# xiuqhou/Salience-DETR

Hardware: AMD Instinct MI355X
Metric: images/s (whole node) + ms/encoder-layer, ResNet50 800x1333 (higher is better)
Workload: dtype bf16; 1 GPU; salience_detr_resnet50_800_1333 bf16 inference, batch=2 per MI355X: pyramid flatten + hierarchical salience filtering + 6-layer salience encoder (MSDA); batch_per_gpu=2, global_batch=2, parallelism=replicas, images sharded across GPUs, no data-path collective, hipgraph=True, hipgraph_nodes=44, hipgraph_memset_nodes=0, world_size=1, backend=none (single process)

## Files before the change

salience_detr_amd/csrc/salience_head.hip:

```cpp
#include <cstdlib>

#include "common.h"

#include "salience_head_core.h"

namespace sdetr {

__global__ void __launch_bounds__(512, 2) salience_head_stage1_x3_kernel(Stage1Args p)
{
    stage1_x3_body(p, (int)blockIdx.x, (int)blockIdx.y);
}

__global__ void __launch_bounds__(512, 2) salience_head_hoist_pyramid_kernel(Stage1Args p, PyramidSrc src, int s1_blocks)
{
    const int blk = (int)blockIdx.x;
    stage1_x3_body<true>(p, blk % s1_blocks, blk / s1_blocks, &src);
}

template <int RT, int WAVES = 4>
__global__ void __launch_bounds__(64 * WAVES, WAVES == 8 ? 2 : (RT == 2 ? 2 : 4)) salience_head_stage1_kernel(Stage1Args p)
{
    constexpr int TM = 32 * RT, THREADS = 64 * WAVES, CT = 8 / WAVES;
    static_assert(TM * 64 % THREADS == 0 && THREADS % TM == 0, "tile / block shape");
    extern __shared__ __attribute__((aligned(16))) float smem[];
    float *tile = smem;
    float *par = smem + TM * kXS;
    float *srow = par + kParRows * kC;
    const int tid = threadIdx.x, lane = tid & 63, wave = tid >> 6;
    const int b = blockIdx.y, blk = blockIdx.x;
    const int t0 = blk * TM;
    const int nvalid = min(TM, p.n - t0);
    const int n0 = wave * (32 * CT);
    const bool with_enc = p.w_enc != nullptr;

    WeightStream<CT, 4> ws;
    ws.start(with_enc ? p.w_enc : p.w1, kC, kC / 8, n0, lane);

    {
        const float *xb = p.x + (int64_t)b * p.x_batch_stride + (int64_t)t0 * p.x_row_stride;
        constexpr int NL = TM * 64 / THREADS;
        float4 v[NL];
#pragma unroll
        for (int i = 0; i < NL; ++i) {
            const int idx = tid + i * THREADS;
            const int r = idx >> 6, c4 = idx & 63;
            v[i] = *reinterpret_cast<const float4 *>(xb + (int64_t)min(r, nvalid - 1) * p.x_row_stride + c4 * 4);
        }
        if (tid < 256) {
            const int row = tid >> 6, c4 = tid & 63;
            const float *src0 = row == 0 ? p.b_enc : row == 1 ? p.g_enc : row == 2 ? p.beta_enc : p.g1;
            const float *src1 = row == 0 ? p.beta1 : p.b1;
            if (with_enc || row == 3) *reinterpret_cast<float4 *>(par + row * kC + c4 * 4) =
                                          *reinterpret_cast<const float4 *>(src0 + c4 * 4);
            if (row < 2) *reinterpret_cast<float4 *>(par + (4 + row) * kC + c4 * 4) =
                             *reinterpret_cast<const float4 *>(src1 + c4 * 4);
        }
        if (tid < TM) {
            float s = 0.f;
            const int t = min(t0 + tid, p.n - 1);
            if (p.row_scale) {
                s = p.row_scale[(int64_t)b * p.n + t];
            } else if (p.coarse) {
                const int y = t / p.w, x = t - y * p.w;
                const float sh = p.h > 1 ? (float)(p.ch - 1) / (float)(p.h - 1) : 0.f;
                const float sw = p.w > 1 ? (float)(p.cw - 1) / (float)(p.w - 1) : 0.f;
                const float fy = sh * (float)y, fx = sw * (float)x;
                const int y1 = (int)fy, x1 = (int)fx;
                const int yp = y1 < p.ch - 1 ? 1 : 0, xp = x1 < p.cw - 1 ? 1 : 0;
                const float ly = fy - (float)y1, lx = fx - (float)x1;
                const float hy = 1.f - ly, hx = 1.f - lx;
                const float *cm = p.coarse + (int64_t)b * p.ch * p.cw;
                s = hy * (hx * cm[y1 * p.cw + x1] + lx * cm[y1 * p.cw + x1 + xp]) +
                    ly * (hx * cm[(y1 + yp) * p.cw + x1] + lx * cm[(y1 + yp) * p.cw + x1 + xp]);
            }
            srow[tid] = s;
            if (tid == 0) srow[TM] = (p.row_scale || p.coarse) ? (p.alpha ? *p.alpha : 1.f) : 0.f;
        }
#pragma unroll
        for (int i = 0; i < NL; ++i) {
            const int idx = tid + i * THREADS;
            const int r = idx >> 6, c4 = idx & 63;
            *reinterpret_cast<float4 *>(tile + r * kXS + c4 * 4) = r < nvalid ? v[i] : make_float4(0.f, 0.f, 0.f, 0.f);
        }
    }
    __syncthreads();

    f32x16 acc[RT][CT];
    if (with_enc) {
        zero_acc(acc);
        block_gemm<kC, kXS, RT, CT, 4>(tile, ws, lane, acc);
        ws.start(p.w1, kC, kC / 8, n0, lane);
        __syncthreads();
#pragma unroll
        for (int ct = 0; ct < CT; ++ct) {
            const int c = n0 + 32 * ct + (lane & 31);
            const float bias = par[kParBEnc * kC + c];
#pragma unroll
            for (int rt = 0; rt < RT; ++rt)
#pragma unroll
                for (int i = 0; i < 16; ++i) tile[(32 * rt + acc_row(i, lane)) * kXS + c] = acc[rt][ct][i] + bias;
        }
        __syncthreads();
    }

    {
        constexpr int TPR = THREADS / TM, NV = kC / 4 / TPR, CS = 4 * TPR;
        const int r = tid / TPR, q = tid % TPR;
        float *row = tile + r * kXS + 4 * q;
        float4 v[NV];
#pragma unroll
        for (int i = 0; i < NV; ++i) v[i] = *reinterpret_cast<const float4 *>(row + CS * i);
        float mean, rstd;
        if (with_enc) {
            row_stats<NV, TPR>(v, p.eps_enc, mean, rstd);
#pragma unroll
            for (int i = 0; i < NV; ++i)
                v[i] = ln_apply(v[i], mean, rstd, *reinterpret_cast<const float4 *>(par + kParGEnc * kC + CS * i + 4 * q),
                                *reinterpret_cast<const float4 *>(par + kParBetaEnc * kC + CS * i + 4 * q));
            if (p.memory_out && r < nvalid) {
                float *mo = p.memory_out + (int64_t)b * p.mem_batch_stride + (int64_t)(t0 + r) * kC + 4 * q;
#pragma unroll
                for (int i = 0; i < NV; ++i) *reinterpret_cast<float4 *>(mo + CS * i) = v[i];
            }
        }
        const float s = srow[r], a = srow[TM];
        if (a != 0.f) {
#pragma unroll
            for (int i = 0; i < NV; ++i)
                v[i] = make_float4(v[i].x + v[i].x * s * a, v[i].y + v[i].y * s * a, v[i].z + v[i].z * s * a,
                                   v[i].w + v[i].w * s * a);
        }
        row_stats<NV, TPR>(v, p.eps1, mean, rstd);
#pragma unroll
        for (int i = 0; i < NV; ++i)
            *reinterpret_cast<float4 *>(row + CS * i) =
                ln_apply(v[i], mean, rstd, *reinterpret_cast<const float4 *>(par + kParG1 * kC + CS * i + 4 * q),
                         *reinterpret_cast<const float4 *>(par + kParBeta1 * kC + CS * i + 4 * q));
    }
    __syncthreads();

    zero_acc(acc);
    block_gemm<kC, kXS, RT, CT, 4>(tile, ws, lane, acc);
    if (n0 < kHalf) {
        float *zl = p.z_local + ((int64_t)b * p.n + t0) * kHalf;
#pragma unroll
        for (int ct = 0; ct < CT; ++ct) {
            const int c = n0 + 32 * ct + (lane & 31);
            const float bias = par[kParB1 * kC + c];
#pragma unroll
            for (int rt = 0; rt < RT; ++rt)
#pragma unroll
                for (int i = 0; i < 16; ++i) {
                    const int r = 32 * rt + acc_row(i, lane);
                    if (r < nvalid) zl[(int64_t)r * kHalf + c] = gelu_erf(acc[rt][ct][i] + bias);
                }
        }
    } else {
#pragma unroll
        for (int ct = 0; ct < CT; ++ct) {
            const int c = n0 + 32 * ct + (lane & 31);
            const float bias = par[kParB1 * kC + c];
            float s = 0.f;
#pragma unroll
            for (int rt = 0; rt < RT; ++rt)
#pragma unroll
                for (int i = 0; i < 16; ++i) {
                    const int r = 32 * rt + acc_row(i, lane);
                    s += r < nvalid ? gelu_erf(acc[rt][ct][i] + bias) : 0.f;
// ... 88 lines not shown
    const int64_t i = (int64_t)blockIdx.x * blockDim.x + threadIdx.x;
    if (i >= (int64_t)N * K) return;
    const int j = (int)(i & 3), h = (int)((i >> 2) & 1);
    const int64_t rest = i >> 3;
    const int n = (int)(rest % N), S = (int)(rest / N);
    out[i] = w[(int64_t)n * row_stride + 8 * S + 4 * h + j];
}

}

using namespace sdetr;

extern "C" int sdetr_pack_linear_f32(sdetr_stream_t stream, const float *weight, int64_t row_stride, int out_features,
                                     int in_features, float *packed)
{
    if (!weight || !packed) return fail("pack_linear: NULL pointer");
    if (out_features <= 0 || in_features <= 0 || in_features % 8 != 0)
        return fail("pack_linear: in_features must be a positive multiple of 8 (got %d x %d)", out_features, in_features);
    const int64_t total = (int64_t)out_features * in_features;
    hipLaunchKernelGGL(pack_linear_kernel, dim3((unsigned)((total + 255) / 256)), dim3(256), 0,
                       static_cast<hipStream_t>(stream), weight, row_stride, out_features, in_features, packed);
    return check_launch("pack_linear");
}

static int stage1_lds_bytes(int tm) { return (tm * kXS + kParRows * kC + tm + 4) * (int)sizeof(float); }

static int stage1_block_tokens(int batch_size, int tokens)
{
    static const int forced = [] { const char *e = ab_env("SDETR_HEAD_ROWTILES"); return e ? atoi(e) : 0; }();
    (void)batch_size; (void)tokens;
    return forced == 2 ? 64 : 32;
}

extern "C" int sdetr_salience_head_blocks(int batch_size, int tokens)
{
    if (tokens <= 0 || batch_size <= 0) return 0;
    const int tm = stage1_block_tokens(batch_size, tokens);
    return (tokens + tm - 1) / tm;
}

extern "C" int sdetr_salience_head_stage1(sdetr_stream_t stream, const float *x, int64_t x_batch_stride,
                                          int64_t x_row_stride, int batch_size, int tokens, int channels,
                                          const float *enc_weight_packed, const float *enc_bias,
                                          const float *enc_norm_weight, const float *enc_norm_bias, float enc_norm_eps,
                                          const float *row_scale, const float *coarse_score, int coarse_h, int coarse_w,
                                          int level_h, int level_w, const float *alpha, const float *norm_weight,
                                          const float *norm_bias, float norm_eps, const float *weight_packed,
                                          const float *bias, float *memory_out, int64_t memory_batch_stride,
                                          float *z_local, float *partial_sums)
{
    if (channels != kC) return fail("salience_head_stage1: built for embed_dim = hidden_dim = %d (got %d)", kC, channels);
    if (batch_size < 0 || tokens < 0) return fail("salience_head_stage1: negative size");
    if (batch_size == 0 || tokens == 0) return 0;
    if (!x || !norm_weight || !norm_bias || !weight_packed || !bias || !z_local || !partial_sums)
        return fail("salience_head_stage1: NULL pointer");
    if (enc_weight_packed && (!enc_bias || !enc_norm_weight || !enc_norm_bias))
        return fail("salience_head_stage1: enc_output parameters incomplete");
    if (row_scale && coarse_score) return fail("salience_head_stage1: give row_scale OR coarse_score");
    if (coarse_score && ((int64_t)level_h * level_w != tokens || coarse_h <= 0 || coarse_w <= 0))
        return fail("salience_head_stage1: level %dx%d does not cover %d tokens", level_h, level_w, tokens);
    if ((x_row_stride % 4) || (x_batch_stride % 4)) return fail("salience_head_stage1: rows must be 16-byte aligned");
    Stage1Args a;
    a.x = x; a.x_batch_stride = x_batch_stride; a.x_row_stride = x_row_stride;
    a.w_enc = reinterpret_cast<const float4 *>(enc_weight_packed);
    a.b_enc = enc_bias; a.g_enc = enc_norm_weight; a.beta_enc = enc_norm_bias; a.eps_enc = enc_norm_eps;
    a.row_scale = row_scale; a.coarse = coarse_score; a.ch = coarse_h; a.cw = coarse_w; a.h = level_h; a.w = level_w;
    a.alpha = alpha; a.g1 = norm_weight; a.beta1 = norm_bias; a.eps1 = norm_eps;
    a.w1 = reinterpret_cast<const float4 *>(weight_packed); a.b1 = bias;
    a.memory_out = enc_weight_packed ? memory_out : nullptr; a.mem_batch_stride = memory_batch_stride;
    a.z_local = z_local; a.partial = partial_sums; a.n = tokens; a.nblk = 0;

    hipStream_t s = static_cast<hipStream_t>(stream);
    if (stage1_block_tokens(batch_size, tokens) == 64) {
        static DeviceOnce lds_once;
        allow_dynamic_lds(salience_head_stage1_kernel<2, 4>, lds_once, (int)stage1_lds_bytes(64));
        a.nblk = (tokens + 63) / 64;
        hipLaunchKernelGGL((salience_head_stage1_kernel<2, 4>), dim3((unsigned)a.nblk, (unsigned)batch_size), dim3(kBlock),
                           (size_t)stage1_lds_bytes(64), s, a);
    } else {
        a.nblk = (tokens + 31) / 32;
        hipLaunchKernelGGL((salience_head_stage1_kernel<1, 8>), dim3((unsigned)a.nblk, (unsigned)batch_size), dim3(512),
                           (size_t)stage1_lds_bytes(32), s, a);
    }
    return check_launch("salience_head_stage1");
}

extern "C" int sdetr_pack_linear_bf16x3(sdetr_stream_t stream, const float *weight, int64_t row_stride, int out_features,
                                        int in_features, void *packed)
{
    if (!weight || !packed) return fail("pack_linear_bf16x3: NULL pointer");
    if (out_features <= 0 || in_features <= 0 || in_features % 16 != 0 || out_features % 32 != 0)
        return fail("pack_linear_bf16x3: [out,in] must be multiples of (32,16) (got %d x %d)", out_features, in_features);
    const int64_t total = (int64_t)out_features * in_features;
    hipLaunchKernelGGL(pack_linear_bf16x3_kernel, dim3((unsigned)((total + 255) / 256)), dim3(256), 0,
                       static_cast<hipStream_t>(stream), weight, row_stride, out_features, in_features,
                       static_cast<uint16_t *>(packed));
    return check_launch("pack_linear_bf16x3");
}

static int stage1_x3_lds_bytes() { return kX3Region + (kParRows * kC + 32 + 4) * (int)sizeof(float); }

extern "C" int sdetr_salience_head_stage1_x3(sdetr_stream_t stream, const float *x, int64_t x_batch_stride,
                                             int64_t x_row_stride, int batch_size, int tokens, int channels,
                                             const void *enc_weight_x3, const float *enc_bias,
                                             const float *enc_norm_weight, const float *enc_norm_bias, float enc_norm_eps,
                                             const float *row_scale, const float *coarse_score, int coarse_h, int coarse_w,
                                             int level_h, int level_w, const float *alpha, const float *norm_weight,
                                             const float *norm_bias, float norm_eps, const void *weight_x3,
                                             const float *bias, float *memory_out, int64_t memory_batch_stride,
                                             float *z_local, float *partial_sums)
{
    if (channels != kC) return fail("salience_head_stage1_x3: built for embed_dim = hidden_dim = %d (got %d)", kC, channels);
    if (batch_size < 0 || tokens < 0) return fail("salience_head_stage1_x3: negative size");
    if (batch_size == 0 || tokens == 0) return 0;
    if (!x || !norm_weight || !norm_bias || !weight_x3 || !bias || !z_local || !partial_sums)
        return fail("salience_head_stage1_x3: NULL pointer");
    if (enc_weight_x3 && (!enc_bias || !enc_norm_weight || !enc_norm_bias))
        return fail("salience_head_stage1_x3: enc_output parameters incomplete");
    if (row_scale && coarse_score) return fail("salience_head_stage1_x3: give row_scale OR coarse_score");
    if (coarse_score && ((int64_t)level_h * level_w != tokens || coarse_h <= 0 || coarse_w <= 0))
        return fail("salience_head_stage1_x3: level %dx%d does not cover %d tokens", level_h, level_w, tokens);
    if ((x_row_stride % 4) || (x_batch_stride % 4)) return fail("salience_head_stage1_x3: rows must be 16-byte aligned");
    if (stage1_block_tokens(batch_size, tokens) != 32)
        return fail("salience_head_stage1_x3: 32-token blocks only (unset SDETR_HEAD_ROWTILES)");
    Stage1Args a;
    a.x = x; a.x_batch_stride = x_batch_stride; a.x_row_stride = x_row_stride;
    a.w_enc = reinterpret_cast<const float4 *>(enc_weight_x3);
    a.b_enc = enc_bias; a.g_enc = enc_norm_weight; a.beta_enc = enc_norm_bias; a.eps_enc = enc_norm_eps;
    a.row_scale = row_scale; a.coarse = coarse_score; a.ch = coarse_h; a.cw = coarse_w; a.h = level_h; a.w = level_w;
    a.alpha = alpha; a.g1 = norm_weight; a.beta1 = norm_bias; a.eps1 = norm_eps;
    a.w1 = reinterpret_cast<const float4 *>(weight_x3); a.b1 = bias;
    a.memory_out = enc_weight_x3 ? memory_out : nullptr; a.mem_batch_stride = memory_batch_stride;
    a.z_local = z_local; a.partial = partial_sums; a.n = tokens; a.nblk = (tokens + 31) / 32;
    hipLaunchKernelGGL(salience_head_stage1_x3_kernel, dim3((unsigned)a.nblk, (unsigned)batch_size), dim3(512),
                       (size_t)stage1_x3_lds_bytes(), static_cast<hipStream_t>(stream), a);
    return check_launch("salience_head_stage1_x3");
}

extern "C" int sdetr_salience_head_hoist_pyramid_x3(
    sdetr_stream_t stream, int num_levels, const float *const *feats, const float *const *pos, const uint8_t *const *masks,
    const int *heights, const int *widths, const float *level_embeds, int batch_size, int channels, int spatial_size,
    uint8_t *mask_out, void *feat_act, void *pos_act, float *valid_ratios, const void *enc_weight_x3, const float *enc_bias,
    const float *enc_norm_weight, const float *enc_norm_bias, float enc_norm_eps, const float *norm_weight,
    const void *weight_x3, float *memory_out, int64_t memory_batch_stride, float *g_out, int64_t g_batch_stride,
    float *sigma_out, int64_t sigma_batch_stride)
{
    if (num_levels <= 0 || num_levels > kPyrMaxLevels) return fail("salience_head_hoist_pyramid_x3: 1..%d levels", kPyrMaxLevels);
    if (channels != kC) return fail("salience_head_hoist_pyramid_x3: built for embed_dim = hidden_dim = %d (got %d)", kC, channels);
    if (batch_size < 0 || spatial_size <= 0) return fail("salience_head_hoist_pyramid_x3: bad dims");
    if (!feats || !pos || !masks || !heights || !widths || !level_embeds || !mask_out || !feat_act || !pos_act)
        return fail("salience_head_hoist_pyramid_x3: null pointer");
    if (!enc_weight_x3 || !enc_bias || !enc_norm_weight || !enc_norm_bias || !norm_weight || !weight_x3 || !g_out || !sigma_out)
        return fail("salience_head_hoist_pyramid_x3: null pointer (head)");
    if ((g_batch_stride % 4) || g_batch_stride < (int64_t)spatial_size * kC || sigma_batch_stride < spatial_size ||
        (memory_out && ((memory_batch_stride % 4) || memory_batch_stride < (int64_t)spatial_size * kC)))
        return fail("salience_head_hoist_pyramid_x3: bad output batch strides");
    if (stage1_block_tokens(batch_size, spatial_size) != 32)
        return fail("salience_head_hoist_pyramid_x3: 32-token blocks only (unset SDETR_HEAD_ROWTILES)");
    PyramidSrc src{};
    src.levels = num_levels;
    int64_t start = 0;
    for (int l = 0; l < num_levels; ++l) {
        const int H = heights[l], W = widths[l];
        if (H <= 0 || W <= 0 || !feats[l] || !pos[l] || !masks[l]) return fail("salience_head_hoist_pyramid_x3: bad level %d", l);
        src.feat[l] = feats[l]; src.pos[l] = pos[l]; src.mask[l] = masks[l];
        src.H[l] = H; src.W[l] = W; src.start[l] = (int)start;
        src.box_wh[l] = 0.05f * (float)(1u << l);
        start += (int64_t)H * W;
        if (start > spatial_size || (int64_t)batch_size * kC * H * W > 0x7fffffffffffLL)
            return fail("salience_head_hoist_pyramid_x3: sizes out of range");
    }
    if (start != spatial_size)
        return fail("salience_head_hoist_pyramid_x3: spatial_size %d is not the pixel count %lld", spatial_size, (long long)start);
    for (int l = num_levels; l <= kPyrMaxLevels; ++l) src.start[l] = spatial_size;
    for (int l = 0; l + kPyrTileLevels < num_levels; ++l)
        if (src.start[l + kPyrTileLevels] / 32 == (src.start[l + 1] - 1) / 32)
            return fail("salience_head_hoist_pyramid_x3: more than %d levels inside one 32-token tile", kPyrTileLevels);
    if (batch_size == 0) return 0;
    src.level_embed = level_embeds;
    src.feat_act = reinterpret_cast<bf16_t *>(feat_act); src.pos_act = reinterpret_cast<bf16_t *>(pos_act);
    src.mask_out = mask_out; src.valid_ratios = valid_ratios;
    Stage1Args a;
    a.x = nullptr; a.x_batch_stride = 0; a.x_row_stride = 0;
    a.w_enc = reinterpret_cast<const float4 *>(enc_weight_x3);
    a.b_enc = enc_bias; a.g_enc = enc_norm_weight; a.beta_enc = enc_norm_bias; a.eps_enc = enc_norm_eps;
    a.row_scale = nullptr; a.coarse = nullptr; a.ch = a.cw = a.h = a.w = 0;
    a.alpha = nullptr; a.g1 = norm_weight; a.beta1 = norm_weight; a.eps1 = 0.f;
    a.w1 = reinterpret_cast<const float4 *>(weight_x3); a.b1 = norm_weight;
    a.memory_out = memory_out; a.mem_batch_stride = memory_batch_stride;
    a.z_local = nullptr; a.partial = nullptr; a.n = spatial_size; a.nblk = (spatial_size + 31) / 32;
    a.g_out = g_out; a.g_batch_stride = g_batch_stride; a.sigma_out = sigma_out; a.sigma_batch_stride = sigma_batch_stride;
    if ((int64_t)a.nblk * batch_size > 0x7fffffff) return fail("salience_head_hoist_pyramid_x3: too many tiles");
    static DeviceOnce lds_once;
    const int lds = kPyrLdsFloats * (int)sizeof(float);
    allow_dynamic_lds(salience_head_hoist_pyramid_kernel, lds_once, lds);
    hipLaunchKernelGGL(salience_head_hoist_pyramid_kernel, dim3((unsigned)(a.nblk * batch_size)), dim3(512), (size_t)lds,
                       static_cast<hipStream_t>(stream), a, src, a.nblk);
    return check_launch("salience_head_hoist_pyramid_x3");
}

extern "C" int sdetr_salience_head_const(sdetr_stream_t stream, const float *partial_sums, int batch_size, int tokens,
                                         const float *weight2, const float *bias2, float *const_workspace,
                                         float *score_min)
{
    if (batch_size < 0 || tokens < 0) return fail("salience_head_const: negative size");
    if (batch_size == 0 || tokens == 0) return 0;
    if (!partial_sums || !weight2 || !bias2 || !const_workspace) return fail("salience_head_const: NULL pointer");
    hipLaunchKernelGGL(salience_head_const_kernel, dim3((unsigned)batch_size), dim3(kHalf * kConstGroups), 0,
                       static_cast<hipStream_t>(stream), partial_sums, sdetr_salience_head_blocks(batch_size, tokens),
                       tokens, weight2, bias2, const_workspace, score_min);
    return check_launch("salience_head_const");
}

extern "C" int sdetr_salience_head_stage2(sdetr_stream_t stream, const float *z_local, const float *partial_sums,
                                          int batch_size, int tokens, const float *weight2, const float *bias2,
                                          const float *weight2_local_packed, const float *weight3_packed,
                                          const float *bias3, const float *weight4, const float *bias4,
                                          float *const_workspace, float *score, float *score_flat,
                                          int64_t score_flat_stride, float *score_min, const void *weight2_local_x3,
                                          int const_in_block)
{
    if (batch_size < 0 || tokens < 0) return fail("salience_head_stage2: negative size");
    if (batch_size == 0 || tokens == 0) return 0;
    if (!z_local || !partial_sums || !weight2 || !bias2 || (!weight2_local_packed && !weight2_local_x3) || !weight3_packed ||
        !bias3 || !weight4 || !bias4 || (!const_workspace && !const_in_block) || !score)
        return fail("salience_head_stage2: NULL pointer");
    const int nblk = (tokens + kTM - 1) / kTM;
    const int prow = sdetr_salience_head_blocks(batch_size, tokens);
    if (const_in_block && prow > kConstInBlockRows)
        return fail("salience_head_stage2: the constant in the block takes up to %d rows of partial sums (got %d)", kConstInBlockRows, prow);
    hipStream_t s = static_cast<hipStream_t>(stream);
    Stage2Args a;
    if (const_in_block) {
        a.partial = partial_sums; a.partial_rows = prow; a.w2 = weight2; a.b2 = bias2;
    } else {
        hipLaunchKernelGGL(salience_head_const_kernel, dim3((unsigned)batch_size), dim3(kHalf * kConstGroups), 0, s,
                           partial_sums, prow, tokens, weight2, bias2, const_workspace, score_min);
        int rc = check_launch("salience_head_const");
        if (rc) return rc;
    }
    a.z_local = z_local; a.cst = const_workspace;
    a.w2a = reinterpret_cast<const float4 *>(weight2_local_packed);
    a.w2a_x3 = weight2_local_x3;
    a.w3 = reinterpret_cast<const float4 *>(weight3_packed);
    a.b3 = bias3; a.w4 = weight4; a.b4 = bias4; a.score = score; a.score2 = score_flat;
    a.score2_stride = score_flat_stride; a.n = tokens; a.score_min = score_min;
    hipLaunchKernelGGL(salience_head_stage2_kernel, dim3((unsigned)nblk, (unsigned)batch_size), dim3(kBlock), 0, s, a);
    return check_launch("salience_head_stage2");
}
```

salience_detr_amd/csrc/salience_head_core.h:

```cpp
#pragma once
#include "common.h"

#pragma clang fp contract(off)

namespace sdetr {

constexpr int kC = 256;
constexpr int kHalf = 128;
constexpr int kTM = 64;
constexpr int kXS = kC + 4;
constexpr int kZS = kHalf + 4;

using f32x16 = __attribute__((ext_vector_type(16))) float;

__device__ __forceinline__ float erf_pos(float t)
{
    float p = 4.535823973128572e-05f;
    p = fmaf(p, t, -0.00044550452730618417f);
    p = fmaf(p, t, 0.0014894308988004923f);
    p = fmaf(p, t, 0.0007746480405330658f);
    p = fmaf(p, t, -0.028253698721528053f);
    p = fmaf(p, t, 0.14848162233829498f);
    p = fmaf(p, t, 0.9184163808822632f);
    p = fmaf(p, t, 1.6279085874557495f);
// ... 60 lines not shown
            if (S + PD < NS) {
#pragma unroll
                for (int ct = 0; ct < CT; ++ct)
                    ws.bq[u][ct] = __builtin_amdgcn_raw_buffer_load_b128(ws.rs, (int)(ws.lane_off + ct * 1024),
                                                                         (int)((S + PD) * ws.step), 0);
            }
#pragma unroll
            for (int rt = 0; rt < RT; ++rt) a[rt] = *reinterpret_cast<const float4 *>(ap + rt * 32 * XS + 8 * S);
            __builtin_amdgcn_sched_barrier(0);
#pragma unroll
            for (int rt = 0; rt < RT; ++rt)
#pragma unroll
                for (int ct = 0; ct < CT; ++ct) {
                    const float4 bf = make_float4(__uint_as_float(b[ct].x), __uint_as_float(b[ct].y),
                                                  __uint_as_float(b[ct].z), __uint_as_float(b[ct].w));
                    acc[rt][ct] = mfma4(a[rt], bf, acc[rt][ct]);
                }
        }
    }
}

template <int RT, int CT>
__device__ __forceinline__ void zero_acc(f32x16 (&acc)[RT][CT])
{
#pragma unroll
    for (int rt = 0; rt < RT; ++rt)
#pragma unroll
        for (int ct = 0; ct < CT; ++ct)
#pragma unroll
            for (int i = 0; i < 16; ++i) acc[rt][ct][i] = 0.f;
}

__device__ __forceinline__ int acc_row(int reg, int lane) { return (reg & 3) + 8 * (reg >> 2) + 4 * (lane >> 5); }

struct Stage1Args {
    const float *x;
    int64_t x_batch_stride, x_row_stride;
    const float4 *w_enc;
    const float *b_enc, *g_enc, *beta_enc;
    float eps_enc;
    const float *row_scale;
    const float *coarse;
    int ch, cw, h, w;
    const float *alpha;
    const float *g1, *beta1;
    float eps1;
    const float4 *w1;
    const float *b1;
    float *memory_out;
    int64_t mem_batch_stride;
    float *z_local;
    float *partial;
    int n, nblk;
    float *g_out = nullptr;
    int64_t g_batch_stride = 0;
    float *sigma_out = nullptr;
    int64_t sigma_batch_stride = 0;
};

template <int TPR>
__device__ __forceinline__ float row_sum(float s)
{
#ifndef SH_SHUFFLE_STATS
    if (TPR == 16) {
        s += __int_as_float(__builtin_amdgcn_update_dpp(0, __float_as_int(s), 0xB1, 0xf, 0xf, true));
        s += __int_as_float(__builtin_amdgcn_update_dpp(0, __float_as_int(s), 0x4E, 0xf, 0xf, true));
        const int t = __builtin_amdgcn_update_dpp(0, __float_as_int(s), 0x141, 0xf, 0xf, true);
        s += __int_as_float(__builtin_amdgcn_update_dpp(0, t, 0x1B, 0xf, 0xf, true));
        s += __int_as_float(__builtin_amdgcn_update_dpp(0, __float_as_int(s), 0x128, 0xf, 0xf, true));
        return s;
    }
#endif
#pragma unroll
    for (int o = 1; o < TPR; o <<= 1) s += __shfl_xor(s, o, TPR);
    return s;
}

template <int NV, int TPR>
__device__ __forceinline__ void row_stats(const float4 (&v)[NV], float eps, float &mean, float &rstd)
{
    float s = 0.f;
#pragma unroll
    for (int i = 0; i < NV; ++i) s += (v[i].x + v[i].y) + (v[i].z + v[i].w);
    s = row_sum<TPR>(s);
    mean = s * (1.f / kC);
    float q = 0.f;
#pragma unroll
    for (int i = 0; i < NV; ++i) {
        const float a = v[i].x - mean, b = v[i].y - mean, c = v[i].z - mean, d = v[i].w - mean;
        q += (a * a + b * b) + (c * c + d * d);
    }
    q = row_sum<TPR>(q);
    rstd = rsqrtf(q * (1.f / kC) + eps);
}

__device__ __forceinline__ float4 ln_apply(float4 v, float mean, float rstd, float4 g, float4 be)
{
    return make_float4((v.x - mean) * rstd * g.x + be.x, (v.y - mean) * rstd * g.y + be.y,
                       (v.z - mean) * rstd * g.z + be.z, (v.w - mean) * rstd * g.w + be.w);
}

enum { kParBEnc = 0, kParGEnc, kParBetaEnc, kParG1, kParBeta1, kParB1, kParRows };


typedef __bf16 sh_bf16x8_t __attribute__((ext_vector_type(8)));
constexpr int kX3Depth = 5;
constexpr int kPlaneRow = kC * 2 + 16;
constexpr int kPlaneBytes = 32 * kPlaneRow;
constexpr int kX3Region = 3 * kPlaneBytes;
static_assert(kX3Region >= 32 * kXS * 4, "the fp32 tile aliases the planes");

__device__ __forceinline__ f32x16 mfma_bf16(u32x4_t a, u32x4_t b, f32x16 c)
{
    return __builtin_amdgcn_mfma_f32_32x32x16_bf16(__builtin_bit_cast(sh_bf16x8_t, a), __builtin_bit_cast(sh_bf16x8_t, b), c, 0, 0, 0);
}

template <bool SOFT>
__device__ __forceinline__ void split3(const float4 v, uint2 &p0, uint2 &p1, uint2 &p2)
{
    if (SOFT) {
    const float x[4] = {v.x, v.y, v.z, v.w};
    uint32_t h[4], m[4], l[4];
#pragma unroll
    for (int i = 0; i < 4; ++i) {
        h[i] = f32_to_bf16_bits(x[i]);
        const float r1 = x[i] - __uint_as_float(h[i] << 16);
        m[i] = f32_to_bf16_bits(r1);
        const float r2 = r1 - __uint_as_float(m[i] << 16);
        l[i] = f32_to_bf16_bits(r2);
    }
    p0 = make_uint2(h[0] | (h[1] << 16), h[2] | (h[3] << 16));
    p1 = make_uint2(m[0] | (m[1] << 16), m[2] | (m[3] << 16));
    p2 = make_uint2(l[0] | (l[1] << 16), l[2] | (l[3] << 16));
    return;
    }
    const uint32_t h01 = pack_bf16x2(v.x, v.y), h23 = pack_bf16x2(v.z, v.w);
    const float r0 = v.x - bf16_lo(h01), r1 = v.y - bf16_hi(h01), r2 = v.z - bf16_lo(h23), r3 = v.w - bf16_hi(h23);
    const uint32_t m01 = pack_bf16x2(r0, r1), m23 = pack_bf16x2(r2, r3);
    const float s0 = r0 - bf16_lo(m01), s1 = r1 - bf16_hi(m01), s2 = r2 - bf16_lo(m23), s3 = r3 - bf16_hi(m23);
    p0 = make_uint2(h01, h23);
    p1 = make_uint2(m01, m23);
    p2 = make_uint2(pack_bf16x2(s0, s1), pack_bf16x2(s2, s3));
}
template <bool SOFT = false>
__device__ __forceinline__ void store_split(char *planes, int row, int col, const float4 v)
{
    uint2 p0, p1, p2;
    split3<SOFT>(v, p0, p1, p2);
    char *d = planes + row * kPlaneRow + col * 2;
    *reinterpret_cast<uint2 *>(d) = p0;
    *reinterpret_cast<uint2 *>(d + kPlaneBytes) = p1;
    *reinterpret_cast<uint2 *>(d + 2 * kPlaneBytes) = p2;
}

template <int PD>
struct WeightStreamX3 {
    __amdgpu_buffer_rsrc_t rs;
    uint32_t lane_off;
    u32x4_t bq[PD][3];
    static constexpr uint32_t kStep = 8 * 3 * 1024;

    __device__ __forceinline__ void start(const void *wp, int ctile, int lane)
    {
        rs = make_uniform_rsrc(reinterpret_cast<const char *>(wp), kStep * (kC / 16));
        lane_off = (uint32_t)(ctile * 3 * 1024 + lane * 16);
#pragma unroll
        for (int u = 0; u < PD; ++u)
#pragma unroll
            for (int pl = 0; pl < 3; ++pl)
                bq[u][pl] = __builtin_amdgcn_raw_buffer_load_b128(rs, (int)(lane_off + pl * 1024), (int)(u * kStep), 0);
    }
};

template <int PD>
__device__ __forceinline__ void block_gemm_x3(const char *planes, WeightStreamX3<PD> &ws, int lane, f32x16 &acc)
{
    constexpr int NS = kC / 16;
    const char *ap = planes + (lane & 31) * kPlaneRow + (lane >> 5) * 16;
#pragma unroll
    for (int S = 0; S < NS; ++S) {
        const int u = S % PD;
        u32x4_t b[3], a[3];
#pragma unroll
        for (int pl = 0; pl < 3; ++pl) b[pl] = ws.bq[u][pl];
        if (S + PD < NS) {
#pragma unroll
            for (int pl = 0; pl < 3; ++pl)
                ws.bq[u][pl] = __builtin_amdgcn_raw_buffer_load_b128(ws.rs, (int)(ws.lane_off + pl * 1024),
                                                                     (int)((S + PD) * ws.kStep), 0);
        }
#pragma unroll
        for (int pl = 0; pl < 3; ++pl) a[pl] = *reinterpret_cast<const u32x4_t *>(ap + pl * kPlaneBytes + S * 32);
        __builtin_amdgcn_sched_barrier(0);
        acc = mfma_bf16(a[2], b[0], acc);
        acc = mfma_bf16(a[0], b[2], acc);
        acc = mfma_bf16(a[1], b[1], acc);
        acc = mfma_bf16(a[1], b[0], acc);
        acc = mfma_bf16(a[0], b[1], acc);
        acc = mfma_bf16(a[0], b[0], acc);
    }
}

template <int NT, int PD>
struct WeightStreamX3G {
    __amdgpu_buffer_rsrc_t rs;
    uint32_t lane_off;
    u32x4_t bq[PD][3];
    static constexpr uint32_t kStep = NT * 3 * 1024;

    __device__ __forceinline__ void start(const void *wp, int ksteps, int ctile, int lane)
    {
        rs = make_uniform_rsrc(reinterpret_cast<const char *>(wp), kStep * (uint32_t)ksteps);
        lane_off = (uint32_t)(ctile * 3 * 1024 + lane * 16);
#pragma unroll
        for (int u = 0; u < PD; ++u)
#pragma unroll
            for (int pl = 0; pl < 3; ++pl)
                bq[u][pl] = __builtin_amdgcn_raw_buffer_load_b128(rs, (int)(lane_off + pl * 1024), (int)(u * kStep), 0);
    }
};
template <int KDIM, int ROWS, int RT, int NT, int PD>
__device__ __forceinline__ void block_gemm_x3g(const char *planes, WeightStreamX3G<NT, PD> &ws, int lane, f32x16 (&acc)[RT])
{
    constexpr int NS = KDIM / 16, kRow = KDIM * 2 + 16, kPlane = ROWS * kRow;
    const char *ap = planes + (lane & 31) * kRow + (lane >> 5) * 16;
#pragma unroll
    for (int S = 0; S < NS; ++S) {
        const int u = S % PD;
        u32x4_t b[3], a[RT][3];
#pragma unroll
        for (int pl = 0; pl < 3; ++pl) b[pl] = ws.bq[u][pl];
        if (S + PD < NS) {
#pragma unroll
            for (int pl = 0; pl < 3; ++pl)
                ws.bq[u][pl] = __builtin_amdgcn_raw_buffer_load_b128(ws.rs, (int)(ws.lane_off + pl * 1024),
                                                                     (int)((S + PD) * ws.kStep), 0);
        }
#pragma unroll
        for (int rt = 0; rt < RT; ++rt)
#pragma unroll
            for (int pl = 0; pl < 3; ++pl)
                a[rt][pl] = *reinterpret_cast<const u32x4_t *>(ap + rt * 32 * kRow + pl * kPlane + S * 32);
        __builtin_amdgcn_sched_barrier(0);
#pragma unroll
        for (int rt = 0; rt < RT; ++rt) {
            acc[rt] = mfma_bf16(a[rt][2], b[0], acc[rt]);
            acc[rt] = mfma_bf16(a[rt][0], b[2], acc[rt]);
            acc[rt] = mfma_bf16(a[rt][1], b[1], acc[rt]);
            acc[rt] = mfma_bf16(a[rt][1], b[0], acc[rt]);
            acc[rt] = mfma_bf16(a[rt][0], b[1], acc[rt]);
            acc[rt] = mfma_bf16(a[rt][0], b[0], acc[rt]);
        }
    }
}
constexpr int kS2PlaneRow = kHalf * 2 + 16;
constexpr int kS2PlaneBytes = 64 * kS2PlaneRow;
constexpr int kS2Planes = 3 * kS2PlaneBytes;

constexpr int kPyrMaxLevels = 8;
constexpr int kPyrTileLevels = 4;
struct PyramidSrc {
    const float *feat[kPyrMaxLevels], *pos[kPyrMaxLevels];
    const uint8_t *mask[kPyrMaxLevels];
    int H[kPyrMaxLevels], W[kPyrMaxLevels], start[kPyrMaxLevels + 1];
    float box_wh[kPyrMaxLevels];
    const float *level_embed;
    int levels;
    bf16_t *feat_act, *pos_act;
    uint8_t *mask_out;
    float *valid_ratios;
};
constexpr int kPyrGeo = 8;
constexpr int kPyrLdsFloats = 2 * 32 * kXS + kParRows * kC + 32 + 4 + kPyrTileLevels * kC + kPyrTileLevels * kPyrGeo + 32 * 4;

template <bool PYR = false>
__device__ __forceinline__ void stage1_x3_body(const Stage1Args &p, int blk, int b, const PyramidSrc *src = nullptr)
{
    constexpr int TM = 32, THREADS = 512;
    extern __shared__ __attribute__((aligned(16))) float smem[];
    char *planes = reinterpret_cast<char *>(smem);
    float *tile = smem;
    float *par = smem + (PYR ? 2 * TM * kXS : kX3Region / 4);
    float *srow = par + kParRows * kC;
    float *tpos = smem + TM * kXS;
    float *lemb = srow + TM + 4;
    float *geo = lemb + kPyrTileLevels * kC;
    int *rowinfo = reinterpret_cast<int *>(geo + kPyrTileLevels * kPyrGeo);
    const int tid = threadIdx.x, lane = tid & 63;
    const int wave = __builtin_amdgcn_readfirstlane(tid >> 6);
    const int t0 = blk * TM;
    const int nvalid = min(TM, p.n - t0);
    const int n0 = wave * 32;
    const bool with_enc = p.w_enc != nullptr;
    const bool hoist = p.g_out != nullptr;

#ifdef SH_STAMPS
    long long sh_t[8];
    int sh_n = 0;
#define SH_STAMP() sh_t[sh_n++] = clock64()
#else
#define SH_STAMP()
#endif
    SH_STAMP();
    WeightStreamX3<kX3Depth> ws;
    ws.start(with_enc ? (const void *)p.w_enc : (const void *)p.w1, wave, lane);

    int l0 = 0;
    {
        constexpr int NL = TM * 64 / THREADS;
        float4 v[NL];
        constexpr int NC = kC * TM / THREADS;
        float pf[NC], pq[NC];
        const int tok = tid & 31, cg = tid >> 5;
        if (PYR) {
            const PyramidSrc &s = *src;
            for (int j = 1; j < s.levels; ++j) l0 += t0 >= s.start[j] ? 1 : 0;
            const int t = min(t0 + tok, p.n - 1);
            int slot = 0, wl = s.W[l0], hw = s.H[l0] * s.W[l0], st = s.start[l0];
            const float *fp = s.feat[l0], *pp = s.pos[l0];
            const uint8_t *mp = s.mask[l0];
#pragma unroll
            for (int k = 1; k < kPyrTileLevels; ++k) {
                const int l = min(l0 + k, s.levels - 1);
                if (l0 + k < s.levels && t >= s.start[l]) {
                    slot = k; wl = s.W[l]; hw = s.H[l] * s.W[l]; st = s.start[l];
                    fp = s.feat[l]; pp = s.pos[l]; mp = s.mask[l];
                }
            }
            const int tl = t - st;
            const int64_t e0 = ((int64_t)b * kC + cg) * hw + tl;
#pragma unroll
            for (int i = 0; i < NC; ++i) pf[i] = fp[e0 + (int64_t)(i * (THREADS / TM)) * hw];
#pragma unroll
            for (int i = 0; i < NC; ++i) pq[i] = pp[e0 + (int64_t)(i * (THREADS / TM)) * hw];
            if (tid < TM) {
                const int y = tl / wl;
                *reinterpret_cast<int4 *>(rowinfo + 4 * tok) = make_int4(slot, tl - y * wl, y, (int)mp[(int64_t)b * hw + tl]);
            }
            {
                const int l = l0 + (wave >> 1);
                if (l < s.levels && s.start[l] < t0 + TM) {
                    const int H = s.H[l], W = s.W[l];
                    const uint8_t *mb = s.mask[l] + (int64_t)b * H * W;
                    int cnt = 0;
                    if (wave & 1) { for (int i = lane; i < W; i += 64) cnt += mb[i] == 0; }
                    else          { for (int i = lane; i < H; i += 64) cnt += mb[(int64_t)i * W] == 0; }
#pragma unroll
                    for (int o = 32; o > 0; o >>= 1) cnt += __shfl_xor(cnt, o);
                    if (lane == 0) {
                        float *g = geo + (wave >> 1) * kPyrGeo;
                        g[wave & 1] = (float)cnt;
                        if (!(wave & 1)) { g[2] = (float)H; g[3] = (float)W; g[4] = s.box_wh[l]; }
                    }
                }
            }
            if (tid >= 256) {
                const int l = l0 + ((tid - 256) >> 6), c4 = tid & 63;
                if (l < s.levels)
                    *reinterpret_cast<float4 *>(lemb + ((tid - 256) >> 6) * kC + c4 * 4) =
                        *reinterpret_cast<const float4 *>(s.level_embed + (int64_t)l * kC + c4 * 4);
            }
        } else {
        const float *xb = p.x + (int64_t)b * p.x_batch_stride + (int64_t)t0 * p.x_row_stride;
#pragma unroll
        for (int i = 0; i < NL; ++i) {
            const int idx = tid + i * THREADS;
            const int r = idx >> 6, c4 = idx & 63;
            v[i] = *reinterpret_cast<const float4 *>(xb + (int64_t)min(r, nvalid - 1) * p.x_row_stride + c4 * 4);
        }
        }
        if (tid < 256) {
            const int row = tid >> 6, c4 = tid & 63;
            const float *src0 = row == 0 ? p.b_enc : row == 1 ? p.g_enc : row == 2 ? p.beta_enc : p.g1;
            const float *src1 = row == 0 ? p.beta1 : p.b1;
            if (with_enc || row == 3) *reinterpret_cast<float4 *>(par + row * kC + c4 * 4) =
                                          *reinterpret_cast<const float4 *>(src0 + c4 * 4);
            if (row < 2) *reinterpret_cast<float4 *>(par + (4 + row) * kC + c4 * 4) =
                             *reinterpret_cast<const float4 *>(src1 + c4 * 4);
        }
        if (tid < TM) {
            float s = 0.f;
            const int t = min(t0 + tid, p.n - 1);
            if (p.row_scale) {
                s = p.row_scale[(int64_t)b * p.n + t];
            } else if (p.coarse) {
                const int y = t / p.w, x = t - y * p.w;
                const float sh = p.h > 1 ? (float)(p.ch - 1) / (float)(p.h - 1) : 0.f;
                const float sw = p.w > 1 ? (float)(p.cw - 1) / (float)(p.w - 1) : 0.f;
                const float fy = sh * (float)y, fx = sw * (float)x;
                const int y1 = (int)fy, x1 = (int)fx;
                const int yp = y1 < p.ch - 1 ? 1 : 0, xp = x1 < p.cw - 1 ? 1 : 0;
                const float ly = fy - (float)y1, lx = fx - (float)x1;
                const float hy = 1.f - ly, hx = 1.f - lx;
                const float *cm = p.coarse + (int64_t)b * p.ch * p.cw;
                s = hy * (hx * cm[y1 * p.cw + x1] + lx * cm[y1 * p.cw + x1 + xp]) +
                    ly * (hx * cm[(y1 + yp) * p.cw + x1] + lx * cm[(y1 + yp) * p.cw + x1 + xp]);
            }
            srow[tid] = s;
            if (tid == 0) srow[TM] = (p.row_scale || p.coarse) ? (p.alpha ? *p.alpha : 1.f) : 0.f;
        }
        if (PYR) {
#pragma unroll
            for (int i = 0; i < NC; ++i) {
                tile[tok * kXS + cg + i * (THREADS / TM)] = pf[i];
                tpos[tok * kXS + cg + i * (THREADS / TM)] = pq[i];
            }
        }
#pragma unroll
        for (int i = 0; i < (PYR ? 0 : NL); ++i) {
            const int idx = tid + i * THREADS;
            const int r = idx >> 6, c4 = idx & 63;
            const float4 val = r < nvalid ? v[i] : make_float4(0.f, 0.f, 0.f, 0.f);
#ifndef SH_SITE1_SOFT
#define SH_SITE1_SOFT false
#endif
#ifndef SH_SITE2_SOFT
#define SH_SITE2_SOFT false
#endif
            if (with_enc) store_split<SH_SITE1_SOFT>(planes, r, c4 * 4, val);
            else *reinterpret_cast<float4 *>(tile + r * kXS + c4 * 4) = val;
        }
    }
#ifdef SH_STAMPS
    asm volatile("s_waitcnt vmcnt(0) lgkmcnt(0)" ::: "memory");
    const long long sh_tile_done = clock64();
#endif
    if (PYR) {
        __syncthreads();
        const PyramidSrc &s = *src;
        const int r = tid >> 4, q = tid & 15;
        const int4 ri = *reinterpret_cast<const int4 *>(rowinfo + 4 * r);
        const float *g = geo + ri.x * kPyrGeo;
        const float vh = g[0], vw = g[1], box_wh = g[4];
        const bool pad = ri.w != 0;
        const float cx = ((float)ri.y + 0.5f) / vw, cy = ((float)ri.z + 0.5f) / vh;
        const bool keep = !pad && cx > 0.01f && cx < 0.99f && cy > 0.01f && cy < 0.99f && box_wh > 0.01f && box_wh < 0.99f;
        const bool live = r < nvalid;
        const int64_t o = ((int64_t)b * p.n + t0 + r) * kC + 4 * q;
        float4 sum[4];
#pragma unroll
        for (int i = 0; i < 4; ++i) {
            const int c = 64 * i + 4 * q;
            const float4 fv = *reinterpret_cast<const float4 *>(tile + r * kXS + c);
            const float4 pv = *reinterpret_cast<const float4 *>(tpos + r * kXS + c);
            const float4 e = *reinterpret_cast<const float4 *>(lemb + ri.x * kC + c);
            const float4 qv = make_float4(pv.x + e.x, pv.y + e.y, pv.z + e.z, pv.w + e.w);
            sum[i] = keep && live ? make_float4(fv.x + qv.x, fv.y + qv.y, fv.z + qv.z, fv.w + qv.w)
                                  : make_float4(0.f, 0.f, 0.f, 0.f);
            if (live) {
                *reinterpret_cast<uint2 *>(s.feat_act + o + 64 * i) = make_uint2(pack_act2(fv.x, fv.y), pack_act2(fv.z, fv.w));
                *reinterpret_cast<uint2 *>(s.pos_act + o + 64 * i) = make_uint2(pack_act2(qv.x, qv.y), pack_act2(qv.z, qv.w));
            }
        }
        if (live && q == 0) {
            s.mask_out[(int64_t)b * p.n + t0 + r] = pad ? 1 : 0;
            if (s.valid_ratios && ri.y == 0 && ri.z == 0) {
                float *vr = s.valid_ratios + ((int64_t)b * s.levels + l0 + ri.x) * 2;
                vr[0] = vw / g[3];
                vr[1] = vh / g[2];
            }
        }
        __syncthreads();
#pragma unroll
        for (int i = 0; i < 4; ++i) store_split<SH_SITE1_SOFT>(planes, r, 64 * i + 4 * q, sum[i]);
    }
    __syncthreads();
    SH_STAMP();

    f32x16 acc;
    if (with_enc) {
#pragma unroll
        for (int i = 0; i < 16; ++i) acc[i] = 0.f;
        block_gemm_x3<kX3Depth>(planes, ws, lane, acc);
        SH_STAMP();
        ws.start(p.w1, wave, lane);
        __syncthreads();
        const int c = n0 + (lane & 31);
        const float bias = par[kParBEnc * kC + c];
#pragma unroll
        for (int i = 0; i < 16; ++i) tile[acc_row(i, lane) * kXS + c] = acc[i] + bias;
        __syncthreads();
        SH_STAMP();
    }

    {
        constexpr int TPR = THREADS / TM, NV = kC / 4 / TPR, CS = 4 * TPR;
        const int r = tid / TPR, q = tid % TPR;
        const float *row = tile + r * kXS + 4 * q;
        float4 v[NV];
#pragma unroll
        for (int i = 0; i < NV; ++i) v[i] = *reinterpret_cast<const float4 *>(row + CS * i);
        float mean, rstd;
        if (with_enc) {
            row_stats<NV, TPR>(v, p.eps_enc, mean, rstd);
#pragma unroll
            for (int i = 0; i < NV; ++i)
                v[i] = ln_apply(v[i], mean, rstd, *reinterpret_cast<const float4 *>(par + kParGEnc * kC + CS * i + 4 * q),
                                *reinterpret_cast<const float4 *>(par + kParBetaEnc * kC + CS * i + 4 * q));
            if (p.memory_out && r < nvalid) {
                float *mo = p.memory_out + (int64_t)b * p.mem_batch_stride + (int64_t)(t0 + r) * kC + 4 * q;
#pragma unroll
                for (int i = 0; i < NV; ++i) *reinterpret_cast<float4 *>(mo + CS * i) = v[i];
            }
        }
        const float s = srow[r], a = srow[TM];
        if (a != 0.f) {
#pragma unroll
            for (int i = 0; i < NV; ++i)
                v[i] = make_float4(v[i].x + v[i].x * s * a, v[i].y + v[i].y * s * a, v[i].z + v[i].z * s * a,
                                   v[i].w + v[i].w * s * a);
        }
        row_stats<NV, TPR>(v, hoist ? 0.f : p.eps1, mean, rstd);
        if (hoist) {
            const bool flat = !(rstd < 3.0e38f);
            if (q == 0 && r < nvalid) p.sigma_out[(int64_t)b * p.sigma_batch_stride + t0 + r] = flat ? 0.f : 1.f / rstd;
            if (flat) rstd = 0.f;
        }
#ifndef SH_NO_PIN_STATS
        asm volatile("" : "+v"(mean), "+v"(rstd));
#endif
#pragma unroll
        for (int i = 0; i < NV; ++i)
            v[i] = ln_apply(v[i], mean, rstd, *reinterpret_cast<const float4 *>(par + kParG1 * kC + CS * i + 4 * q),
                            hoist ? make_float4(0.f, 0.f, 0.f, 0.f)
                                  : *reinterpret_cast<const float4 *>(par + kParBeta1 * kC + CS * i + 4 * q));
        asm volatile("s_waitcnt lgkmcnt(0)" ::: "memory");
        __builtin_amdgcn_sched_barrier(0);
        __syncthreads();
#pragma unroll
        for (int i = 0; i < NV; ++i) store_split<SH_SITE2_SOFT>(planes, r, CS * i + 4 * q, v[i]);
    }
    __syncthreads();
    SH_STAMP();

#pragma unroll
    for (int i = 0; i < 16; ++i) acc[i] = 0.f;
    block_gemm_x3<kX3Depth>(planes, ws, lane, acc);
    SH_STAMP();
    if (hoist) {
        const int c = n0 + (lane & 31);
        float *g = p.g_out + (int64_t)b * p.g_batch_stride + (int64_t)t0 * kC + c;
#pragma unroll
        for (int i = 0; i < 16; ++i) {
            const int r = acc_row(i, lane);
            if (r < nvalid) g[(int64_t)r * kC] = acc[i];
        }
    } else {
        const int c = n0 + (lane & 31);
        const float bias = par[kParB1 * kC + c];
        if (n0 < kHalf) {
            float *zl = p.z_local + ((int64_t)b * p.n + t0) * kHalf;
#pragma unroll
            for (int i = 0; i < 16; ++i) {
                const int r = acc_row(i, lane);
                if (r < nvalid) zl[(int64_t)r * kHalf + c] = gelu_erf(acc[i] + bias);
            }
        } else {
            float s = 0.f;
#pragma unroll
            for (int i = 0; i < 16; ++i) s += acc_row(i, lane) < nvalid ? gelu_erf(acc[i] + bias) : 0.f;
            s += __shfl_xor(s, 32);
            if (lane < 32) p.partial[((int64_t)b * p.nblk + blk) * kHalf + (c - kHalf)] = s;
        }
    }
#ifdef SH_STAMPS
    SH_STAMP();
    if (with_enc && tid == 0 && b == 0 && (blk == 0 || blk == p.nblk / 2 || blk == p.nblk - 1))
        printf("stage1 n=%d blk=%d cycles: (own part of the tile %lld) tile %lld | gemm1 %lld | to-lds %lld | ln %lld | gemm2 %lld | epilogue %lld | total %lld\n", p.n, blk,
               sh_tile_done - sh_t[0], sh_t[1] - sh_t[0], sh_t[2] - sh_t[1], sh_t[3] - sh_t[2], sh_t[4] - sh_t[3], sh_t[5] - sh_t[4], sh_t[6] - sh_t[5], sh_t[6] - sh_t[0]);
#endif
}

struct ModulateArgs {
    const float *g;
    int64_t g_batch_stride;
    const float *sigma;
    int64_t sigma_batch_stride;
    const float *row_scale;
    const float *coarse;
    int ch, cw, h, w;
    const float *alpha;
    float eps1;
    const float *c0;
    float *z_local;
    float *partial;
    int n, nblk;
    float *score_min_init;
};

constexpr int kModThreads = 256;
constexpr int kModLdsFloats = 32 + 4 * kHalf;

__device__ __forceinline__ void modulate_body(const ModulateArgs &p, int blk, int b, float *lds, int tid)
{
    constexpr int TM = 32;
    float *kk = lds, *red = lds + 32;
    const int lane = tid & 63, wave = tid >> 6;
    const int t0 = blk * TM;
    const int nvalid = min(TM, p.n - t0);
    if (p.score_min_init && blk == 0 && b == 0 && tid == 0) *p.score_min_init = INFINITY;
    float sg = 0.f, v00 = 0.f, v01 = 0.f, v10 = 0.f, v11 = 0.f, ly = 0.f, lx = 0.f;
    const bool modulated = p.row_scale || p.coarse;
    if (tid < TM) {
        const int t = min(t0 + tid, p.n - 1);
        sg = p.sigma[(int64_t)b * p.sigma_batch_stride + t];
        if (p.row_scale) {
            v00 = p.row_scale[(int64_t)b * p.n + t];
        } else if (p.coarse) {
            const int y = t / p.w, x = t - y * p.w;
            const float sh = p.h > 1 ? (float)(p.ch - 1) / (float)(p.h - 1) : 0.f;
            const float sw = p.w > 1 ? (float)(p.cw - 1) / (float)(p.w - 1) : 0.f;
            const float fy = sh * (float)y, fx = sw * (float)x;
            const int y1 = (int)fy, x1 = (int)fx;
            const int yp = y1 < p.ch - 1 ? 1 : 0, xp = x1 < p.cw - 1 ? 1 : 0;
            ly = fy - (float)y1;
            lx = fx - (float)x1;
            const float *cm = p.coarse + (int64_t)b * p.ch * p.cw;
// ... 232 lines not shown
```

Baseline: 2062 images/s.

## Swizzle pyramid LDS tile, widen activation stores, and deal blocks XCD-contiguously

In the pyramid-hoist head kernel, block indices are remapped so consecutive tiles land on the same XCD for L2 locality. The LDS transpose writes are XOR-swizzled per token group to cut bank conflicts, and the reads unswizzle them. The bf16 feature and position activation stores widen from 8-byte to 16-byte per lane, and the split-plane LDS stores widen the same way. A new host check requires 16-byte alignment of the activation outputs, and compile flags can restore the old paths.

```diff
diff --git a/salience_detr_amd/csrc/salience_head.hip b/salience_detr_amd/csrc/salience_head.hip
--- a/salience_detr_amd/csrc/salience_head.hip
+++ b/salience_detr_amd/csrc/salience_head.hip
@@ -11,9 +11,20 @@
     stage1_x3_body(p, (int)blockIdx.x, (int)blockIdx.y);
 }
 
+__device__ __forceinline__ int xcd_contiguous_tile(int i, int n)
+{
+    constexpr int kXcds = 8;
+    const int x = i % kXcds, base = n / kXcds, rem = n % kXcds;
+    return x * base + min(x, rem) + i / kXcds;
+}
+
 __global__ void __launch_bounds__(512, 2) salience_head_hoist_pyramid_kernel(Stage1Args p, PyramidSrc src, int s1_blocks)
 {
+#ifdef SH_NO_XCD_DEAL
     const int blk = (int)blockIdx.x;
+#else
+    const int blk = xcd_contiguous_tile((int)blockIdx.x, (int)gridDim.x);
+#endif
     stage1_x3_body<true>(p, blk % s1_blocks, blk / s1_blocks, &src);
 }
 
@@ -408,6 +419,8 @@
         return fail("salience_head_hoist_pyramid_x3: null pointer");
     if (!enc_weight_x3 || !enc_bias || !enc_norm_weight || !enc_norm_bias || !norm_weight || !weight_x3 || !g_out || !sigma_out)
         return fail("salience_head_hoist_pyramid_x3: null pointer (head)");
+    if ((reinterpret_cast<uintptr_t>(feat_act) | reinterpret_cast<uintptr_t>(pos_act)) & 15)
+        return fail("salience_head_hoist_pyramid_x3: feat_act / pos_act must be 16-byte aligned");
     if ((g_batch_stride % 4) || g_batch_stride < (int64_t)spatial_size * kC || sigma_batch_stride < spatial_size ||
         (memory_out && ((memory_batch_stride % 4) || memory_batch_stride < (int64_t)spatial_size * kC)))
         return fail("salience_head_hoist_pyramid_x3: bad output batch strides");
diff --git a/salience_detr_amd/csrc/salience_head_core.h b/salience_detr_amd/csrc/salience_head_core.h
--- a/salience_detr_amd/csrc/salience_head_core.h
+++ b/salience_detr_amd/csrc/salience_head_core.h
@@ -236,6 +236,17 @@
     *reinterpret_cast<uint2 *>(d + kPlaneBytes) = p1;
     *reinterpret_cast<uint2 *>(d + 2 * kPlaneBytes) = p2;
 }
+template <bool SOFT = false>
+__device__ __forceinline__ void store_split8(char *planes, int row, int col, const float4 lo, const float4 hi)
+{
+    uint2 a0, a1, a2, b0, b1, b2;
+    split3<SOFT>(lo, a0, a1, a2);
+    split3<SOFT>(hi, b0, b1, b2);
+    char *d = planes + row * kPlaneRow + col * 2;
+    *reinterpret_cast<uint4 *>(d) = make_uint4(a0.x, a0.y, b0.x, b0.y);
+    *reinterpret_cast<uint4 *>(d + kPlaneBytes) = make_uint4(a1.x, a1.y, b1.x, b1.y);
+    *reinterpret_cast<uint4 *>(d + 2 * kPlaneBytes) = make_uint4(a2.x, a2.y, b2.x, b2.y);
+}
 
 template <int PD>
 struct WeightStreamX3 {
@@ -356,6 +367,20 @@
 };
 constexpr int kPyrGeo = 8;
 constexpr int kPyrLdsFloats = 2 * 32 * kXS + kParRows * kC + 32 + 4 + kPyrTileLevels * kC + kPyrTileLevels * kPyrGeo + 32 * 4;
+__device__ __forceinline__ int pyr_swizzle(int r)
+{
+#ifdef SH_NO_TSWZ
+    return 0;
+#else
+    return (r >> 3) & 3;
+#endif
+}
+__device__ __forceinline__ float4 pyr_unswizzle(float4 v, int sw)
+{
+    if (sw & 1) v = make_float4(v.y, v.x, v.w, v.z);
+    if (sw & 2) v = make_float4(v.z, v.w, v.x, v.y);
+    return v;
+}
 
 template <bool PYR = false>
 __device__ __forceinline__ void stage1_x3_body(const Stage1Args &p, int blk, int b, const PyramidSrc *src = nullptr)
@@ -484,10 +509,11 @@
             if (tid == 0) srow[TM] = (p.row_scale || p.coarse) ? (p.alpha ? *p.alpha : 1.f) : 0.f;
         }
         if (PYR) {
+            const int sw = pyr_swizzle(tok);
 #pragma unroll
             for (int i = 0; i < NC; ++i) {
-                tile[tok * kXS + cg + i * (THREADS / TM)] = pf[i];
-                tpos[tok * kXS + cg + i * (THREADS / TM)] = pq[i];
+                tile[tok * kXS + ((cg + i * (THREADS / TM)) ^ sw)] = pf[i];
+                tpos[tok * kXS + ((cg + i * (THREADS / TM)) ^ sw)] = pq[i];
             }
         }
 #pragma unroll
@@ -520,13 +546,15 @@
         const float cx = ((float)ri.y + 0.5f) / vw, cy = ((float)ri.z + 0.5f) / vh;
         const bool keep = !pad && cx > 0.01f && cx < 0.99f && cy > 0.01f && cy < 0.99f && box_wh > 0.01f && box_wh < 0.99f;
         const bool live = r < nvalid;
+        const int sw = pyr_swizzle(4 * wave);
+#ifdef SH_NO_WIDE_ACT
         const int64_t o = ((int64_t)b * p.n + t0 + r) * kC + 4 * q;
         float4 sum[4];
 #pragma unroll
         for (int i = 0; i < 4; ++i) {
             const int c = 64 * i + 4 * q;
-            const float4 fv = *reinterpret_cast<const float4 *>(tile + r * kXS + c);
-            const float4 pv = *reinterpret_cast<const float4 *>(tpos + r * kXS + c);
+            const float4 fv = pyr_unswizzle(*reinterpret_cast<const float4 *>(tile + r * kXS + c), sw);
+            const float4 pv = pyr_unswizzle(*reinterpret_cast<const float4 *>(tpos + r * kXS + c), sw);
             const float4 e = *reinterpret_cast<const float4 *>(lemb + ri.x * kC + c);
             const float4 qv = make_float4(pv.x + e.x, pv.y + e.y, pv.z + e.z, pv.w + e.w);
             sum[i] = keep && live ? make_float4(fv.x + qv.x, fv.y + qv.y, fv.z + qv.z, fv.w + qv.w)
@@ -536,6 +564,30 @@
                 *reinterpret_cast<uint2 *>(s.pos_act + o + 64 * i) = make_uint2(pack_act2(qv.x, qv.y), pack_act2(qv.z, qv.w));
             }
         }
+#else
+        const int64_t o = ((int64_t)b * p.n + t0 + r) * kC + 8 * q;
+        float4 sum[4];
+#pragma unroll
+        for (int h = 0; h < 2; ++h) {
+            uint32_t fa[4], qa[4];
+#pragma unroll
+            for (int k = 0; k < 2; ++k) {
+                const int c = 128 * h + 8 * q + 4 * k;
+                const float4 fv = pyr_unswizzle(*reinterpret_cast<const float4 *>(tile + r * kXS + c), sw);
+                const float4 pv = pyr_unswizzle(*reinterpret_cast<const float4 *>(tpos + r * kXS + c), sw);
+                const float4 e = *reinterpret_cast<const float4 *>(lemb + ri.x * kC + c);
+                const float4 qv = make_float4(pv.x + e.x, pv.y + e.y, pv.z + e.z, pv.w + e.w);
+                sum[2 * h + k] = keep && live ? make_float4(fv.x + qv.x, fv.y + qv.y, fv.z + qv.z, fv.w + qv.w)
+                                              : make_float4(0.f, 0.f, 0.f, 0.f);
+                fa[2 * k] = pack_act2(fv.x, fv.y); fa[2 * k + 1] = pack_act2(fv.z, fv.w);
+                qa[2 * k] = pack_act2(qv.x, qv.y); qa[2 * k + 1] = pack_act2(qv.z, qv.w);
+            }
+            if (live) {
+                *reinterpret_cast<uint4 *>(s.feat_act + o + 128 * h) = make_uint4(fa[0], fa[1], fa[2], fa[3]);
+                *reinterpret_cast<uint4 *>(s.pos_act + o + 128 * h) = make_uint4(qa[0], qa[1], qa[2], qa[3]);
+            }
+        }
+#endif
         if (live && q == 0) {
             s.mask_out[(int64_t)b * p.n + t0 + r] = pad ? 1 : 0;
             if (s.valid_ratios && ri.y == 0 && ri.z == 0) {
@@ -545,8 +597,13 @@
             }
         }
         __syncthreads();
+#ifdef SH_NO_WIDE_ACT
 #pragma unroll
         for (int i = 0; i < 4; ++i) store_split<SH_SITE1_SOFT>(planes, r, 64 * i + 4 * q, sum[i]);
+#else
+#pragma unroll
+        for (int h = 0; h < 2; ++h) store_split8<SH_SITE1_SOFT>(planes, r, 128 * h + 8 * q, sum[2 * h], sum[2 * h + 1]);
+#endif
     }
     __syncthreads();
     SH_STAMP();
```

Measured after the change: 2061 images/s. About the same (-0.0%).
